# hooman007/ProtoASNet

Measured on AMD Instinct MI355X. Metric: clips/sec forward, higher is better.
Workload: dtype bf16; 1 GPU; Video ProtoASNet forward, x3d_s trunk + prototype layer (P=30, D=256, K=3), 32x16x224x224 echo clips per GPU; global_batch=32, parallelism=dp1 (independent clips, no collective), launch=hipGraph replay of the forward's launch list (one graph launch per step)

## Files before the change

### protoasnet_amd/csrc/stem_mfma.hip

```cpp
#include "common.h"
#include "igemm_epilogue.h"

namespace pasn {

constexpr int SM_ROWS = 4, SM_COLS = 56, SM_PC = 116, SM_PR = 2 * (SM_ROWS - 1) + 3, SM_RING = 6;
static_assert(SM_PC % 4 == 0 && SM_PC >= 2 * SM_COLS + 4, "whole 4-column staging units, every window inside the patch");
constexpr int SM_PF = 3;

template <typename TIN>
struct SmRaw;
template <>
struct SmRaw<float> {
    f32x4 v;
    __device__ void load(const float* p) { v = *reinterpret_cast<const f32x4*>(p); }
    __device__ float get(int e) const { return v[e]; }
};
template <>
struct SmRaw<__bf16> {
    bf16x4 v;
    __device__ void load(const __bf16* p) { v = *reinterpret_cast<const bf16x4*>(p); }
    __device__ float get(int e) const { return (float)v[e]; }
};
template <>
struct SmRaw<unsigned char> {
    unsigned v;
    __device__ void load(const unsigned char* p) { v = *reinterpret_cast<const unsigned*>(p); }
    __device__ float get(int e) const { return (float)((v >> (8 * e)) & 0xffu); }
};

template <typename TIN, int CIN>
__global__ __launch_bounds__(256, 2) void x3d_stem_mfma_kernel(const TIN* __restrict__ x, const __bf16* __restrict__ wq,
                                                               const float* __restrict__ scale, const float* __restrict__ bias,
                                                               __bf16* __restrict__ y, pasn_conv_desc d, float in_a, float in_b) {
    constexpr int NT = 1, MT = 2, BN = 32, OROW = BN + 8;
    constexpr int RPF = CIN * 3;
    constexpr int KROWS = 5 * RPF;
    constexpr int KS = (KROWS + 3) / 4;
    constexpr int SLOT = CIN * SM_PR * SM_PC;
    constexpr int UNITS = SLOT / 4;
    constexpr int UPT = (UNITS + 255) / 256;
    extern __shared__ __attribute__((aligned(16))) char smem[];
    __bf16* const ring = reinterpret_cast<__bf16*>(smem);
    __bf16* const imgs = reinterpret_cast<__bf16*>(smem + SM_RING * SLOT * 2);
    float* const scb = reinterpret_cast<float*>(smem + SM_RING * SLOT * 2 + 4 * 32 * OROW * 2);
    const int tid = threadIdx.x, lane = tid & 63, wave = __builtin_amdgcn_readfirstlane(tid >> 6);
    const int c = lane & 31, h = lane >> 5;
    const int T = d.Ti;

    const int ncol = (d.Wo + SM_COLS - 1) / SM_COLS, nrow = (d.Ho + SM_ROWS - 1) / SM_ROWS;
    int b = blockIdx.x;
    const int ct = b % ncol;
    b /= ncol;
    const int rt = b % nrow;
    const int n = b / nrow;
    const int oh0 = rt * SM_ROWS, ow0 = ct * SM_COLS;
    const int hi_base = oh0 * 2 - 1, wi_base = ow0 * 2 - 4;

    bf16x8 wa[KS];
#pragma unroll
    for (int s = 0; s < KS; ++s) wa[s] = *reinterpret_cast<const bf16x8*>(wq + ((size_t)(2 * s + h) * BN + c) * 8);
    igemm_stage_scale_bias<BN>(scb, scale, bias, 0, d.Cout_p, tid);

    const long plane = (long)d.Hi * d.Wi;
    int uoff[UPT];
    int uci[UPT];
#pragma unroll
    for (int k = 0; k < UPT; ++k) {
        const int u = tid + 256 * k;
        const int pc4 = u % (SM_PC / 4), r = (u / (SM_PC / 4)) % SM_PR, ci = u / ((SM_PC / 4) * SM_PR);
        const int hi = hi_base + r, wi = wi_base + pc4 * 4;
        const bool ok = u < UNITS && (unsigned)hi < (unsigned)d.Hi && (unsigned)wi < (unsigned)d.Wi;
        uoff[k] = ok ? hi * d.Wi + wi : -1;
        uci[k] = ci < CIN ? ci : CIN - 1;
    }
    SmRaw<TIN> raw[UPT];
    auto fetch = [&](int ti) {
#pragma unroll
        for (int k = 0; k < UPT; ++k)
            raw[k].load(x + (((long)n * CIN + uci[k]) * T + ti) * plane + (uoff[k] >= 0 ? uoff[k] : 0));
    };
    auto stage = [&](int slot, bool inside) {
        __bf16* dst = ring + slot * SLOT;
#pragma unroll
        for (int k = 0; k < UPT; ++k) {
            const int u = tid + 256 * k;
            float v[4];
#pragma unroll
            for (int e = 0; e < 4; ++e) v[e] = (inside && uoff[k] >= 0) ? fmaf(raw[k].get(e), in_a, in_b) : 0.0f;
            if (u < UNITS) store4(dst + u * 4, v);
        }
    };

    const int lane_off = (2 * wave) * SM_PC + 2 * c + 2;
    const int oh = oh0 + wave;
    const int cgs = d.Cout_p / 8;
    __bf16* const img = imgs + (size_t)wave * 32 * OROW;

    auto emit = [&](int to, const int (&sb)[5]) {
        f32x16 acc[NT][MT];
#pragma unroll
        for (int j = 0; j < MT; ++j)
#pragma unroll
            for (int r = 0; r < 16; ++r) acc[0][j][r] = 0.0f;
#pragma unroll
        for (int s = 0; s < KS; ++s) {
            auto rowoff = [&](int R) {
                const int Rc = R < KROWS ? R : KROWS - 1;
                return sb[Rc / RPF] + (((Rc % RPF) / 3) * SM_PR + (Rc % RPF) % 3) * SM_PC;
            };
            const int oa = h ? rowoff(4 * s + 2) : rowoff(4 * s + 0);
            const int ob = h ? rowoff(4 * s + 3) : rowoff(4 * s + 1);
            const __bf16* srca = ring + lane_off + oa;
            const __bf16* srcb = ring + lane_off + ob;
            bf16x8 bfr[MT];
#pragma unroll
            for (int j = 0; j < MT; ++j) {
                typedef unsigned u32x4 __attribute__((ext_vector_type(4)));
                const unsigned* pa = reinterpret_cast<const unsigned*>(srca + 64 * j);
                const unsigned* pb = reinterpret_cast<const unsigned*>(srcb + 64 * j);
                u32x4 v;
                v.x = pa[0];
                v.y = pa[1];
                v.z = pb[0];
                v.w = pb[1];
                bfr[j] = __builtin_bit_cast(bf16x8, v);
            }
#pragma unroll
            for (int j = 0; j < MT; ++j) mma32(acc[0][j], wa[s], bfr[j]);
        }
        __builtin_amdgcn_sched_group_barrier(0x100, 2 * MT * SM_PF, 0);
#pragma unroll
        for (int s = 0; s < KS; ++s) {
            __builtin_amdgcn_sched_group_barrier(0x008, MT, 0);
            if (s + SM_PF < KS) __builtin_amdgcn_sched_group_barrier(0x100, 2 * MT, 0);
        }
        igemm_epilogue<NT, MT>(acc, img, scb, nullptr, y, 0, cgs, d, lane, [&](int j, long& mbase, int& nvalid) {
            mbase = (((long)n * d.To + to) * d.Ho + oh) * d.Wo + ow0 + 32 * j;
            nvalid = oh < d.Ho ? min(min(32, SM_COLS - 32 * j), d.Wo - (ow0 + 32 * j)) : 0;
        });
    };

    const int nf = T + 4;
    int r = 0;
#pragma unroll 1
    for (int f = 0; f < nf; ++f) {
        const int ti = f - 2;
        stage(r, ti >= 0 && ti < T);
        if (ti + 1 >= 0 && ti + 1 < T) fetch(ti + 1);
        __syncthreads();
        const int to = f - 4;
        if (to >= 0) {
            int sb[5];
#pragma unroll
            for (int kt = 0; kt < 5; ++kt) {
                int q = r + 2 + kt;
                q = q >= SM_RING ? q - SM_RING : q;
                q = q >= SM_RING ? q - SM_RING : q;
                sb[kt] = q * SLOT;
            }
            emit(to, sb);
        }
        r = r + 1 == SM_RING ? 0 : r + 1;
    }
}

int x3d_stem_mfma_supported(const pasn_conv_desc& d, int out_dtype) {
    if (const char* e = tune("PASN_NO_STEM_MFMA"))
        if (e[0] == '1') return 0;
    if (out_dtype != PASN_BF16 || (d.Cin != 1 && d.Cin != 3) || d.Cout_p > 32) return 0;
    if (d.kt != 1 || d.kh != 3 || d.kw != 3 || d.st != 1 || d.sh != 2 || d.sw != 2 || d.pt != 0 || d.ph != 1 || d.pw != 1) return 0;
    if (d.Wi % 4 != 0 || d.To != d.Ti) return 0;
    if ((long)d.N * d.Cin * d.Ti * d.Hi * d.Wi >= (1L << 31)) return 0;
    return 1;
}

template <typename TIN>
static int launch_stem_mfma_t(const void* x, const void* wq, const float* scale, const float* bias, void* y, const pasn_conv_desc& d,
                              float in_a, float in_b, hipStream_t s) {
    const size_t slot = (size_t)d.Cin * SM_PR * SM_PC * 2;
    const size_t lds = SM_RING * slot + (size_t)4 * 32 * (32 + 8) * 2 + 32 * 8;
    const dim3 grid((unsigned)((long)d.N * ceil_div(d.Ho, SM_ROWS) * ceil_div(d.Wo, SM_COLS))), block(256);
    if (d.Cin == 3) {
        PASN_MAX_LDS(96 * 1024, x3d_stem_mfma_kernel<TIN, 3>);
        hipLaunchKernelGGL((x3d_stem_mfma_kernel<TIN, 3>), grid, block, lds, s, (const TIN*)x, (const __bf16*)wq, scale, bias, (__bf16*)y, d,
                           in_a, in_b);
    } else {
        hipLaunchKernelGGL((x3d_stem_mfma_kernel<TIN, 1>), grid, block, lds, s, (const TIN*)x, (const __bf16*)wq, scale, bias, (__bf16*)y, d,
                           in_a, in_b);
    }
    return check_launch("x3d_stem_mfma_kernel");
}

int launch_x3d_stem_mfma(const void* x, const void* wq, const float* scale, const float* bias, void* y, const pasn_conv_desc& d, int in_dtype,
                         float in_a, float in_b, hipStream_t s) {
    if (in_dtype == PASN_F32) return launch_stem_mfma_t<float>(x, wq, scale, bias, y, d, in_a, in_b, s);
    if (in_dtype == PASN_BF16) return launch_stem_mfma_t<__bf16>(x, wq, scale, bias, y, d, in_a, in_b, s);
    if (in_dtype == PASN_U8) return launch_stem_mfma_t<unsigned char>(x, wq, scale, bias, y, d, in_a, in_b, s);
    set_error("x3d_stem_mfma: unknown input dtype");
    return PASN_ERR_ARG;
}

}
```

### protoasnet_amd/csrc/x3d_edp.hip

```cpp
#include "common.h"
#include "xb_pointwise.h"

namespace pasn {

struct EdpArgs {
    const __bf16* x;
    const __bf16* w_a;
    const float *s_a, *b_a;
    const unsigned short* wq;
    const float *s_dw, *b_dw;
    const __bf16* w_c;
    const float *s_c, *b_c;
    __bf16* y;
    const __bf16* w_n;
    const float *s_n, *b_n;
    __bf16* e_next;
    int N, T, Cm, Cmp, Cxp, Cnp;
};

#ifdef PASN_TUNING
__device__ long long edp_stamps[8];
#define EDP_NOW() ((long long)__builtin_amdgcn_s_memrealtime())
#define EDP_ON (g.stamps && blockIdx.x == 0 && threadIdx.x == 0)
#endif

__device__ __forceinline__ void edp_barrier() { asm volatile("s_waitcnt lgkmcnt(0)\n\ts_barrier" ::: "memory"); }

constexpr int EDP_HW = 7, EDP_S = 49;
constexpr int EDP_RWI = 10, EDP_SLOTS = 10;
constexpr int EDP_ROWP = EDP_RWI * EDP_SLOTS + 2;
constexpr int EDP_FB = 9 * EDP_ROWP * 16;
constexpr int EDP_CPL = 9;

template <int KSA, int KSC, bool NEXT>
__global__ __launch_bounds__(512) void x3d_edp_kernel(EdpArgs a, EdpGeom g) {
    extern __shared__ __attribute__((aligned(1024))) char smem[];
    constexpr int XPL = 2 * KSA + 1;
    constexpr int TF = 2, NF = TF + 2, R = TF * EDP_S, RI = NF * EDP_S;
    const int lane = threadIdx.x & 63, wave = __builtin_amdgcn_readfirstlane(threadIdx.x >> 6);
    const int tid = threadIdx.x;
    const int c = lane & 31, h = lane >> 5;
    const int m = lane & 15, q4 = lane >> 4;
    char* const xin = smem;
    char* const fimg = smem + g.fimg_off;
    char* const dch = smem + g.dch_off;
    char* const xt = fimg;
    unsigned* const rowtab = reinterpret_cast<unsigned*>(smem + g.tab_off);
    float* const cst = reinterpret_cast<float*>(smem + g.cst_off);
    const int Cmp = a.Cmp, Cxp = a.Cxp, T = a.T;
    float* const sdw = cst, *const bdw = cst + Cmp, *const scp = cst + 2 * Cmp, *const bcp = scp + 32 * g.CTC, *const snp = bcp + 32 * g.CTC,
                *const bnp = snp + 32 * g.CTN;

#ifdef PASN_TUNING
    long long te = 0, td = 0, tp = 0, tq = 0;
    if (EDP_ON) edp_stamps[0] = EDP_NOW();
#endif
    for (int i = tid; i < (g.tab_off - g.fimg_off) / 16; i += 512) reinterpret_cast<uint4*>(fimg)[i] = uint4{0u, 0u, 0u, 0u};
    for (int i = tid; i < Cmp; i += 512) {
        sdw[i] = a.s_dw[i];
        bdw[i] = a.b_dw[i];
    }
    for (int i = tid; i < 32 * g.CTC; i += 512) {
        scp[i] = a.s_c[i];
        bcp[i] = a.b_c[i];
    }
    if (NEXT)
        for (int i = tid; i < 32 * g.CTN; i += 512) {
            snp[i] = a.s_n[i];
            bnp[i] = a.b_n[i];
        }
    const long M = (long)a.N * T * EDP_S;
    const __amdgpu_buffer_rsrc_t xrsrc = __builtin_amdgcn_make_buffer_rsrc(const_cast<__bf16*>(a.x), 0, (unsigned)(M * Cxp * 2), 0x00020000);
    const __amdgpu_buffer_rsrc_t yrsrc = __builtin_amdgcn_make_buffer_rsrc(a.y, 0, (unsigned)(M * Cxp * 2), 0x00020000);
    const __amdgpu_buffer_rsrc_t ersrc = __builtin_amdgcn_make_buffer_rsrc(NEXT ? a.e_next : a.y, 0, NEXT ? (unsigned)(M * a.Cnp * 2) : 0u, 0x00020000);
    const int PPR = Cxp >> 3;
    const int nTch = (T + TF - 1) / TF;
    const int lbl = xcd_remap(blockIdx.x, gridDim.x);
    const int tile_end = min(g.tiles, (lbl + 1) * g.tpb);
    const int ctw = wave & 3, tfo = wave >> 2;
    const int mrow = m / EDP_HW, mcol = m - mrow * EDP_HW;
    const int dwsel = (m & 7) >> 1, wsh = (m & 1) * 16;
    int tapoff[5];
#pragma unroll
    for (int j = 0; j < 5; ++j) {
        const int tap9 = min(2 * j + (q4 >> 1), 8);
        tapoff[j] = ((tap9 / 3) * EDP_ROWP + (tap9 % 3) * EDP_SLOTS) * 16;
    }
    const bool mpos = m < 2 * EDP_HW;
    const int lbase0 = ((mpos ? mrow : 1) * EDP_ROWP + (mpos ? mcol : EDP_HW - 1) * EDP_SLOTS + 2 * ctw + (q4 & 1)) * 16;
    constexpr int lstep = 2 * EDP_ROWP * 16;
    const int CT16 = (Cmp + 15) >> 4;
    const int prt = wave & 3, pcg = wave >> 2;
    const int ea = wave & 1, er = wave >> 1;
    __syncthreads();

#pragma unroll 1
    for (int tile = lbl * g.tpb; tile < tile_end; ++tile) {
        const int tch = tile % nTch, n = tile / nTch;
        const int t0 = tch * TF;
        const int nix = (RI * XPL + 63) >> 6;
        for (int j = wave; j < nix; j += 8) {
            const int s = j * 64 + lane;
            const int r = s / XPL, p = s - r * XPL;
            const int f = r / EDP_S, pos = r - f * EDP_S, ti = t0 - 1 + f;
            const unsigned off = (r < RI && p < PPR && ti >= 0 && ti < T) ? (unsigned)(((n * T + ti) * EDP_S + pos) * Cxp + p * 8) * 2u : XB_OOB;
            __builtin_amdgcn_raw_ptr_buffer_load_lds(xrsrc, (xb_lds_ptr_t)(xin + j * 1024), 16, (int)off, 0, 0, 0);
        }
        if (tid < 128) {
            const int f = tid / EDP_S, pos = tid - f * EDP_S;
            rowtab[tid] = (tid < R && t0 + f < T) ? (unsigned)((n * T + t0 + f) * EDP_S + pos) : 0xffffffffu;
        }
        f32x16 pacc[3];
#pragma unroll
        for (int i = 0; i < 3; ++i)
#pragma unroll
            for (int r = 0; r < 16; ++r) pacc[i][r] = 0.0f;
        asm volatile("s_waitcnt vmcnt(0)" ::: "memory");
        __syncthreads();
#ifdef PASN_TUNING
        if (EDP_ON) edp_stamps[1] = EDP_NOW();
#endif

#pragma unroll 1
        for (int qd = 0; qd < g.NQ; ++qd) {
#ifdef PASN_TUNING
            if (g.stamps) tq = EDP_NOW();
#endif
            {
                const int co = min(2 * qd + ea, g.CTA - 1);
                const bool colive = 2 * qd + ea < g.CTA;
                bf16x8 A[KSA];
                const __bf16* ab = a.w_a + ((long)co * KSA * 64 + lane) * 8;
#pragma unroll
                for (int ks = 0; ks < KSA; ++ks) A[ks] = load_frag<__bf16>(ab + ks * 512);
                float scv[2][8], bsv[2][8];
#pragma unroll
                for (int pr = 0; pr < 2; ++pr) {
                    load8(a.s_a + co * 32 + 16 * pr + 8 * h, scv[pr]);
                    load8(a.b_a + co * 32 + 16 * pr + 8 * h, bsv[pr]);
                }
                f32x16 acc[2];
#pragma unroll
                for (int i = 0; i < 2; ++i)
#pragma unroll
                    for (int r = 0; r < 16; ++r) acc[i][r] = 0.0f;
                const char* b0 = xin + ((er * 32 + c) * XPL + h) * 16;
#pragma unroll
                for (int ks = 0; ks < KSA; ++ks) {
                    const bf16x8 B0 = *reinterpret_cast<const bf16x8*>(b0 + ks * 32);
                    const bf16x8 B1 = *reinterpret_cast<const bf16x8*>(b0 + 4 * 32 * XPL * 16 + ks * 32);
                    acc[0] = __builtin_amdgcn_mfma_f32_32x32x16_bf16(A[ks], B0, acc[0], 0, 0, 0);
                    acc[1] = __builtin_amdgcn_mfma_f32_32x32x16_bf16(A[ks], B1, acc[1], 0, 0, 0);
                }
#pragma unroll
                for (int i = 0; i < 2; ++i) {
                    const int r = (er + 4 * i) * 32 + c;
                    const int f = r / EDP_S, pos = r - f * EDP_S;
                    const int ph = pos / EDP_HW, pw = pos - ph * EDP_HW;
                    const int ti = t0 - 1 + f;
                    const bool wr = colive && r < RI;
                    const bool inclip = ti >= 0 && ti < T;
                    char* const cell = wr ? fimg + f * EDP_FB + ((ph + 1) * EDP_ROWP + (pw + 1) * EDP_SLOTS + 4 * ea + h) * 16 : dch + R * EDP_CPL * 16;
#pragma unroll
                    for (int pr = 0; pr < 2; ++pr) {
                        float v[8];
#pragma unroll
                        for (int qq = 0; qq < 4; ++qq) {
                            const auto sw = __builtin_amdgcn_permlane32_swap(__float_as_uint(acc[i][8 * pr + qq]), __float_as_uint(acc[i][8 * pr + 4 + qq]), false, false);
                            v[qq] = __uint_as_float(sw[0]);
                            v[4 + qq] = __uint_as_float(sw[1]);
                        }
#pragma unroll
                        for (int e = 0; e < 8; ++e) v[e] = v[e] * scv[pr][e] + bsv[pr][e];
                        bf16x8 o;
#pragma unroll
                        for (int e = 0; e < 8; ++e) o[e] = (__bf16)relu_f32(v[e]);
                        xb_u32x4 ou = __builtin_bit_cast(xb_u32x4, o);
                        if (!inclip) ou = xb_u32x4{0u, 0u, 0u, 0u};
                        *reinterpret_cast<xb_u32x4*>(cell + (wr ? pr * 32 : 0)) = ou;
                    }
                }
            }
            const int c0 = (qd * 4 + ctw) * 16;
            const bool dlive = c0 < Cmp;
            const int ct = min(qd * 4 + ctw, CT16 - 1);
            const uint4* wp = reinterpret_cast<const uint4*>(a.wq + ((size_t)(ct * 2) * 64 + lane) * 8);
            const uint4 w0v = wp[0], w1v = wp[64];
            bf16x8 PA[3][4];
#pragma unroll
            for (int i = 0; i < 3; ++i)
#pragma unroll
                for (int kk = 0; kk < 4; ++kk)
                    PA[i][kk] = load_frag<__bf16>(a.w_c + ((long)((pcg + 2 * i) * KSC + min(4 * qd + kk, KSC - 1)) * 64 + lane) * 8);
            edp_barrier();
#ifdef PASN_TUNING
            if (g.stamps) {
                const long long now = EDP_NOW();
                te += now - tq;
                tq = now;
            }
#endif
            if (dlive && t0 + tfo < T) {
                xb_u32x4 A[3][5];
                const unsigned wd[8] = {w0v.x, w0v.y, w0v.z, w0v.w, w1v.x, w1v.y, w1v.z, w1v.w};
#pragma unroll
                for (int kt = 0; kt < 3; ++kt)
#pragma unroll
                    for (int j = 0; j < 5; ++j) {
                        const int e = kt * 5 + j;
                        const unsigned bits = ((e & 1) ? (wd[e >> 1] >> 16) : (wd[e >> 1] & 0xffffu)) << wsh;
                        A[kt][j] = xb_u32x4{dwsel == 0 ? bits : 0u, dwsel == 1 ? bits : 0u, dwsel == 2 ? bits : 0u, dwsel == 3 ? bits : 0u};
                    }
                f32x4 S[4];
#pragma unroll
                for (int l = 0; l < 4; ++l) S[l] = f32x4{0.0f, 0.0f, 0.0f, 0.0f};
#pragma unroll
                for (int kt = 0; kt < 3; ++kt) {
                    const char* fb = fimg + (tfo + kt) * EDP_FB + lbase0;
#pragma unroll
                    for (int l = 0; l < 4; ++l) {
                        bf16x8 B[5];
#pragma unroll
                        for (int j = 0; j < 5; ++j) B[j] = *reinterpret_cast<const bf16x8*>(fb + tapoff[j] + l * lstep);
#pragma unroll
                        for (int j = 0; j < 5; ++j) S[l] = __builtin_amdgcn_mfma_f32_16x16x32_bf16(__builtin_bit_cast(bf16x8, A[kt][j]), B[j], S[l], 0, 0, 0);
                    }
                }
                const int ce = c0 + 4 * q4, cel = ctw * 16 + 4 * q4;
                const bool cev = ce < Cmp;
                const f32x4 s4 = *reinterpret_cast<const f32x4*>(sdw + min(ce, Cmp - 4)), b4 = *reinterpret_cast<const f32x4*>(bdw + min(ce, Cmp - 4));
#pragma unroll
                for (int l = 0; l < 4; ++l) {
                    const int lr = 2 * l + mrow;
                    const bool ok = m < 2 * EDP_HW && lr < EDP_HW && cev;
                    float v[4];
#pragma unroll
                    for (int i = 0; i < 4; ++i) {
                        v[i] = S[l][i] * (cev ? s4[i] : 0.0f) + (cev ? b4[i] : 0.0f);
                        v[i] = v[i] * sigmoidf_(v[i]);
                    }
                    bf16x4 o;
#pragma unroll
                    for (int i = 0; i < 4; ++i) o[i] = (__bf16)v[i];
                    const int r = ok ? tfo * EDP_S + lr * EDP_HW + mcol : R;
                    *reinterpret_cast<bf16x4*>(dch + (r * EDP_CPL) * 16 + (ok ? cel : 0) * 2) = o;
                }
            }
            edp_barrier();
#ifdef PASN_TUNING
            if (g.stamps) {
                const long long now = EDP_NOW();
                td += now - tq;
                tq = now;
            }
#endif
            {
                const char* b0 = dch + ((prt * 32 + c) * EDP_CPL + h) * 16;
#pragma unroll
                for (int kk = 0; kk < 4; ++kk) {
                    if (4 * qd + kk < KSC) {
                        const bf16x8 B = *reinterpret_cast<const bf16x8*>(b0 + kk * 32);
#pragma unroll
                        for (int i = 0; i < 3; ++i) pacc[i] = __builtin_amdgcn_mfma_f32_32x32x16_bf16(PA[i][kk], B, pacc[i], 0, 0, 0);
                    }
                }
            }
#ifdef PASN_TUNING
            if (g.stamps) tp += EDP_NOW() - tq;
#endif
        }
#ifdef PASN_TUNING
        if (EDP_ON) {
            edp_stamps[2] = EDP_NOW();
            edp_stamps[5] = te;
            edp_stamps[6] = td;
            edp_stamps[7] = tp;
        }
#endif
        if (NEXT) __syncthreads();
        {
            const int r = prt * 32 + c;
            const unsigned gp = rowtab[r];
#pragma unroll
            for (int i = 0; i < 3; ++i) {
                const int co = pcg + 2 * i;
                unsigned off[2];
                uint4 rraw[2];
#pragma unroll
                for (int pr = 0; pr < 2; ++pr) {
                    const int ch = co * 32 + 16 * pr + 8 * h;
                    off[pr] = (gp != 0xffffffffu && ch < Cxp) ? (gp * (unsigned)Cxp + (unsigned)ch) * 2u : XB_OOB;
                    rraw[pr] = __builtin_bit_cast(uint4, __builtin_amdgcn_raw_buffer_load_b128(xrsrc, (int)off[pr], 0, 0));
                }
#pragma unroll
                for (int pr = 0; pr < 2; ++pr) {
                    float v[8], r8[8], scv[8], bsv[8];
#pragma unroll
                    for (int qq = 0; qq < 4; ++qq) {
                        const auto sw = __builtin_amdgcn_permlane32_swap(__float_as_uint(pacc[i][8 * pr + qq]), __float_as_uint(pacc[i][8 * pr + 4 + qq]), false, false);
                        v[qq] = __uint_as_float(sw[0]);
                        v[4 + qq] = __uint_as_float(sw[1]);
                    }
                    const int ch = co * 32 + 16 * pr + 8 * h;
                    load8(scp + ch, scv);
                    load8(bcp + ch, bsv);
                    const uint4 rr1[1] = {rraw[pr]};
                    raw_to_f8<__bf16>(rr1, r8);
#pragma unroll
                    for (int e = 0; e < 8; ++e) v[e] = v[e] * scv[e] + bsv[e];
#pragma unroll
                    for (int e = 0; e < 8; ++e) v[e] += r8[e];
                    bf16x8 o;
#pragma unroll
                    for (int e = 0; e < 8; ++e) o[e] = (__bf16)relu_f32(v[e]);
                    __builtin_amdgcn_raw_buffer_store_b128(__builtin_bit_cast(xb_u32x4, o), yrsrc, (int)off[pr], 0, 0);
                    if (NEXT && ch < Cxp) *reinterpret_cast<bf16x8*>(xt + (r * XPL + (ch >> 3)) * 16) = o;
                }
            }
        }
#ifdef PASN_TUNING
        if (EDP_ON) edp_stamps[3] = EDP_NOW();
#endif
        if (NEXT) {
            __syncthreads();
            xb_pointwise<KSA, 4, false, false>(a.w_n, snp, bnp, xt, XPL, g.CTN, 4, rowtab, ersrc, ersrc, a.Cnp, nullptr, 0, wave, lane);
            __syncthreads();
#ifdef PASN_TUNING
            if (EDP_ON) edp_stamps[4] = EDP_NOW();
#endif
            for (int i = tid; i < (NF * EDP_FB) / 16; i += 512) reinterpret_cast<uint4*>(fimg)[i] = uint4{0u, 0u, 0u, 0u};
        }
        __syncthreads();
    }
}

static bool edp_pointwise(const pasn_conv_desc& d) {
    return d.kt == 1 && d.kh == 1 && d.kw == 1 && d.st == 1 && d.sh == 1 && d.sw == 1 && !d.pt && !d.ph && !d.pw;
}

EdpGeom edp_geom(const pasn_conv_desc& da, const pasn_conv_desc& dd, const pasn_conv_desc& dc, const pasn_conv_desc* dn, int dtype) {
    EdpGeom g{};
    if (dtype != PASN_BF16) return g;
    if (const char* e = tune("PASN_NO_EDP"))
        if (e[0] == '1') return g;
    const bool stencil = dd.kt == 3 && dd.kh == 3 && dd.kw == 3 && dd.st == 1 && dd.sh == 1 && dd.sw == 1 && dd.pt == 1 && dd.ph == 1 && dd.pw == 1 &&
                         dd.To == dd.Ti && dd.Ho == dd.Hi && dd.Wo == dd.Wi && dd.Cin_p == dd.Cout_p && dd.act == PASN_ACT_SWISH;
    if (!stencil || !edp_pointwise(da) || !edp_pointwise(dc) || da.act != PASN_ACT_RELU || dc.act != PASN_ACT_RELU || da.in_swish || dc.in_swish) return g;
    if (dd.Hi != EDP_HW || dd.Wi != EDP_HW) return g;
    if (da.N != dd.N || da.To != dd.Ti || da.Ho != dd.Hi || da.Wo != dd.Wi || da.Cout != dd.Cin || da.Cout_p != dd.Cin_p) return g;
    if (dc.N != dd.N || dc.To != dd.To || dc.Ho != dd.Ho || dc.Wo != dd.Wo || dc.Cin != dd.Cout || dc.Cin_p != dd.Cout_p) return g;
    if (dc.Cout != da.Cin || dc.Cout_p != da.Cin_p) return g;
    if (da.w_frag != 1 || dc.w_frag != 1 || da.Cin_p != 192 || dd.Cout_p != 432) return g;
    g.KSA = da.Cin_p / 16;
    g.KSC = (dd.Cout_p + 31) / 32 * 2;
    if (da.w_kc != g.KSA * 16 || dc.w_kc != g.KSC * 16) return EdpGeom{};
    g.CTA = (da.Cout_p + 31) / 32;
    g.CTC = (dc.Cout_p + 31) / 32;
    if (g.CTC != 6 || da.w_rows < g.CTA * 32 || dc.w_rows < g.CTC * 32) return EdpGeom{};
    if (dn) {
        if (!edp_pointwise(*dn) || dn->act != PASN_ACT_RELU || dn->in_swish || dn->w_frag != 1) return EdpGeom{};
        if (dn->N != dc.N || dn->To != dc.To || dn->Ho != dc.Ho || dn->Wo != dc.Wo || dn->Cin != dc.Cout || dn->Cin_p != dc.Cout_p) return EdpGeom{};
        g.CTN = (dn->Cout_p + 31) / 32;
        if (dn->w_kc != g.KSA * 16 || dn->w_rows < g.CTN * 32 || dn->Cout_p % 8) return EdpGeom{};
    }
    const long M = (long)dd.N * dd.To * EDP_S;
    if (M * dd.Cout_p * 2 >= (1L << 30) || (dn && M * dn->Cout_p * 2 >= (1L << 30))) return EdpGeom{};
    g.NQ = ceil_div(dd.Cout_p, 64);
    auto kib = [](int b) { return (b + 1023) / 1024 * 1024; };
    const int xpl = 2 * g.KSA + 1;
    g.fimg_off = kib(4 * EDP_S * xpl * 16);
    const int fimg_bytes = kib(std::max(4 * EDP_FB, dn ? 128 * xpl * 16 + 64 : 0));
    g.dch_off = g.fimg_off + fimg_bytes;
    g.tab_off = g.dch_off + kib((2 * EDP_S + 1) * EDP_CPL * 16 + 64);
    g.cst_off = g.tab_off + 1024;
    g.lds_bytes = g.cst_off + kib((2 * dd.Cout_p + 64 * g.CTC + 64 * g.CTN) * 4);
    if (g.lds_bytes > 160 * 1024) return EdpGeom{};
    g.tiles = dd.N * ceil_div(dd.To, 2);
    const int grid = std::min(g.tiles, 256);
    g.tpb = ceil_div(g.tiles, grid);
    g.grid = ceil_div(g.tiles, g.tpb);
    g.stamps = tune_dev("PASN_EDP_STAMPS") ? 1 : 0;
    g.ok = 1;
    return g;
}

}

using namespace pasn;

#ifdef PASN_TUNING
extern "C" int pasn_debug_edp_stamps(long long* host_out) { return (int)hipMemcpyFromSymbol(host_out, HIP_SYMBOL(pasn::edp_stamps), sizeof(long long) * 8); }
#endif

static bool edp_desc_ok(const pasn_conv_desc* d) { return d && d->N > 0 && d->To > 0 && d->Ho > 0 && d->Wo > 0 && d->Cin > 0 && d->Cout > 0; }

extern "C" int pasn_x3d_edp_supported(const pasn_conv_desc* d_a, const pasn_conv_desc* d_dw, const pasn_conv_desc* d_c, const pasn_conv_desc* d_n, int dtype) {
    if (!edp_desc_ok(d_a) || !edp_desc_ok(d_dw) || !edp_desc_ok(d_c) || (d_n && !edp_desc_ok(d_n))) return 0;
    return edp_geom(*d_a, *d_dw, *d_c, d_n, dtype).ok;
}

extern "C" int pasn_x3d_edp_fwd(const void* x, const void* w_a, const float* scale_a, const float* bias_a, const void* w_dw, const float* scale_dw,
                                const float* bias_dw, const void* w_c, const float* scale_c, const float* bias_c, void* y, const void* w_n,
                                const float* scale_n, const float* bias_n, void* e_next, const pasn_conv_desc* d_a, const pasn_conv_desc* d_dw,
                                const pasn_conv_desc* d_c, const pasn_conv_desc* d_n, int dtype, void* stream) {
    PASN_REQUIRE(x && w_a && scale_a && bias_a && w_dw && scale_dw && bias_dw && w_c && scale_c && bias_c && y, "null pointer");
    PASN_REQUIRE((d_n != nullptr) == (w_n != nullptr) && (d_n == nullptr || (scale_n && bias_n && e_next)), "the next expand conv comes with all of its operands, or not at all");
    PASN_REQUIRE(edp_desc_ok(d_a) && edp_desc_ok(d_dw) && edp_desc_ok(d_c) && (!d_n || edp_desc_ok(d_n)), "bad geometry");
    const EdpGeom g = edp_geom(*d_a, *d_dw, *d_c, d_n, dtype);
    PASN_REQUIRE(g.ok, "block not covered (pasn_x3d_edp_supported returns 0)");
    EdpArgs a{(const __bf16*)x, (const __bf16*)w_a, scale_a, bias_a, (const unsigned short*)w_dw, scale_dw, bias_dw, (const __bf16*)w_c, scale_c, bias_c,
              (__bf16*)y, (const __bf16*)w_n, scale_n, bias_n, (__bf16*)e_next, d_dw->N, d_dw->To, d_dw->Cout, d_dw->Cout_p, d_a->Cin_p,
              d_n ? d_n->Cout_p : 0};
    const dim3 grid(g.grid), block(512);
    if (d_n) {
        PASN_MAX_LDS(160 * 1024, x3d_edp_kernel<12, 28, true>);
        hipLaunchKernelGGL((x3d_edp_kernel<12, 28, true>), grid, block, (size_t)g.lds_bytes, (hipStream_t)stream, a, g);
    } else {
        PASN_MAX_LDS(160 * 1024, x3d_edp_kernel<12, 28, false>);
        hipLaunchKernelGGL((x3d_edp_kernel<12, 28, false>), grid, block, (size_t)g.lds_bytes, (hipStream_t)stream, a, g);
    }
    return check_launch("x3d_edp_kernel");
}
```

Before: 12020 clips/s.

## Prime stem ring early, overlap EDP input fetch with setup, reuse staged residual

```diff
diff --git a/protoasnet_amd/csrc/stem_mfma.hip b/protoasnet_amd/csrc/stem_mfma.hip
--- a/protoasnet_amd/csrc/stem_mfma.hip
+++ b/protoasnet_amd/csrc/stem_mfma.hip
@@ -48,7 +48,7 @@
     const int T = d.Ti;
 
     const int ncol = (d.Wo + SM_COLS - 1) / SM_COLS, nrow = (d.Ho + SM_ROWS - 1) / SM_ROWS;
-    int b = blockIdx.x;
+    int b = xcd_remap(blockIdx.x, gridDim.x);
     const int ct = b % ncol;
     b /= ncol;
     const int rt = b % nrow;
@@ -74,12 +74,12 @@
         uci[k] = ci < CIN ? ci : CIN - 1;
     }
     SmRaw<TIN> raw[UPT];
-    auto fetch = [&](int ti) {
+    auto fetch = [&](SmRaw<TIN>(&raw)[UPT], int ti) {
 #pragma unroll
         for (int k = 0; k < UPT; ++k)
             raw[k].load(x + (((long)n * CIN + uci[k]) * T + ti) * plane + (uoff[k] >= 0 ? uoff[k] : 0));
     };
-    auto stage = [&](int slot, bool inside) {
+    auto stage = [&](const SmRaw<TIN>(&raw)[UPT], int slot, bool inside) {
         __bf16* dst = ring + slot * SLOT;
 #pragma unroll
         for (int k = 0; k < UPT; ++k) {
@@ -140,16 +140,25 @@
         });
     };
 
+    static_assert((4 * SLOT) % 16 == 0, "slots 0 and 1 cleared in 16-byte units");
+    for (int i = tid; i < (4 * SLOT) / 16; i += 256) reinterpret_cast<uint4*>(ring)[i] = uint4{0u, 0u, 0u, 0u};
+    {
+        SmRaw<TIN> raw0[UPT], raw1[UPT];
+        fetch(raw0, 0);
+        if (1 < T) fetch(raw1, 1);
+        if (2 < T) fetch(raw, 2);
+        stage(raw0, 2, true);
+        stage(raw1, 3, 1 < T);
+        stage(raw, 4, 2 < T);
+    }
+    if (3 < T) fetch(raw, 3);
+    __syncthreads();
     const int nf = T + 4;
-    int r = 0;
+    int r = 4;
 #pragma unroll 1
-    for (int f = 0; f < nf; ++f) {
-        const int ti = f - 2;
-        stage(r, ti >= 0 && ti < T);
-        if (ti + 1 >= 0 && ti + 1 < T) fetch(ti + 1);
-        __syncthreads();
-        const int to = f - 4;
-        if (to >= 0) {
+    for (int f = 4;;) {
+        {
+            const int to = f - 4;
             int sb[5];
 #pragma unroll
             for (int kt = 0; kt < 5; ++kt) {
@@ -161,6 +170,11 @@
             emit(to, sb);
         }
         r = r + 1 == SM_RING ? 0 : r + 1;
+        if (++f == nf) break;
+        const int ti = f - 2;
+        stage(raw, r, ti < T);
+        if (ti + 1 < T) fetch(raw, ti + 1);
+        __syncthreads();
     }
 }
 
diff --git a/protoasnet_amd/csrc/x3d_edp.hip b/protoasnet_amd/csrc/x3d_edp.hip
--- a/protoasnet_amd/csrc/x3d_edp.hip
+++ b/protoasnet_amd/csrc/x3d_edp.hip
@@ -55,20 +55,6 @@
     long long te = 0, td = 0, tp = 0, tq = 0;
     if (EDP_ON) edp_stamps[0] = EDP_NOW();
 #endif
-    for (int i = tid; i < (g.tab_off - g.fimg_off) / 16; i += 512) reinterpret_cast<uint4*>(fimg)[i] = uint4{0u, 0u, 0u, 0u};
-    for (int i = tid; i < Cmp; i += 512) {
-        sdw[i] = a.s_dw[i];
-        bdw[i] = a.b_dw[i];
-    }
-    for (int i = tid; i < 32 * g.CTC; i += 512) {
-        scp[i] = a.s_c[i];
-        bcp[i] = a.b_c[i];
-    }
-    if (NEXT)
-        for (int i = tid; i < 32 * g.CTN; i += 512) {
-            snp[i] = a.s_n[i];
-            bnp[i] = a.b_n[i];
-        }
     const long M = (long)a.N * T * EDP_S;
     const __amdgpu_buffer_rsrc_t xrsrc = __builtin_amdgcn_make_buffer_rsrc(const_cast<__bf16*>(a.x), 0, (unsigned)(M * Cxp * 2), 0x00020000);
     const __amdgpu_buffer_rsrc_t yrsrc = __builtin_amdgcn_make_buffer_rsrc(a.y, 0, (unsigned)(M * Cxp * 2), 0x00020000);
@@ -76,26 +62,8 @@
     const int PPR = Cxp >> 3;
     const int nTch = (T + TF - 1) / TF;
     const int lbl = xcd_remap(blockIdx.x, gridDim.x);
-    const int tile_end = min(g.tiles, (lbl + 1) * g.tpb);
-    const int ctw = wave & 3, tfo = wave >> 2;
-    const int mrow = m / EDP_HW, mcol = m - mrow * EDP_HW;
-    const int dwsel = (m & 7) >> 1, wsh = (m & 1) * 16;
-    int tapoff[5];
-#pragma unroll
-    for (int j = 0; j < 5; ++j) {
-        const int tap9 = min(2 * j + (q4 >> 1), 8);
-        tapoff[j] = ((tap9 / 3) * EDP_ROWP + (tap9 % 3) * EDP_SLOTS) * 16;
-    }
-    const bool mpos = m < 2 * EDP_HW;
-    const int lbase0 = ((mpos ? mrow : 1) * EDP_ROWP + (mpos ? mcol : EDP_HW - 1) * EDP_SLOTS + 2 * ctw + (q4 & 1)) * 16;
-    constexpr int lstep = 2 * EDP_ROWP * 16;
-    const int CT16 = (Cmp + 15) >> 4;
-    const int prt = wave & 3, pcg = wave >> 2;
-    const int ea = wave & 1, er = wave >> 1;
-    __syncthreads();
-
-#pragma unroll 1
-    for (int tile = lbl * g.tpb; tile < tile_end; ++tile) {
+    const int tile0 = lbl * g.tpb, tile_end = min(g.tiles, (lbl + 1) * g.tpb);
+    auto request_x = [&](int tile) {
         const int tch = tile % nTch, n = tile / nTch;
         const int t0 = tch * TF;
         const int nix = (RI * XPL + 63) >> 6;
@@ -110,6 +78,43 @@
             const int f = tid / EDP_S, pos = tid - f * EDP_S;
             rowtab[tid] = (tid < R && t0 + f < T) ? (unsigned)((n * T + t0 + f) * EDP_S + pos) : 0xffffffffu;
         }
+    };
+    if (tile0 < tile_end) request_x(tile0);
+    for (int i = tid; i < (g.tab_off - g.fimg_off) / 16; i += 512) reinterpret_cast<uint4*>(fimg)[i] = uint4{0u, 0u, 0u, 0u};
+    for (int i = tid; i < Cmp; i += 512) {
+        sdw[i] = a.s_dw[i];
+        bdw[i] = a.b_dw[i];
+    }
+    for (int i = tid; i < 32 * g.CTC; i += 512) {
+        scp[i] = a.s_c[i];
+        bcp[i] = a.b_c[i];
+    }
+    if (NEXT)
+        for (int i = tid; i < 32 * g.CTN; i += 512) {
+            snp[i] = a.s_n[i];
+            bnp[i] = a.b_n[i];
+        }
+    const int ctw = wave & 3, tfo = wave >> 2;
+    const int mrow = m / EDP_HW, mcol = m - mrow * EDP_HW;
+    const int dwsel = (m & 7) >> 1, wsh = (m & 1) * 16;
+    int tapoff[5];
+#pragma unroll
+    for (int j = 0; j < 5; ++j) {
+        const int tap9 = min(2 * j + (q4 >> 1), 8);
+        tapoff[j] = ((tap9 / 3) * EDP_ROWP + (tap9 % 3) * EDP_SLOTS) * 16;
+    }
+    const bool mpos = m < 2 * EDP_HW;
+    const int lbase0 = ((mpos ? mrow : 1) * EDP_ROWP + (mpos ? mcol : EDP_HW - 1) * EDP_SLOTS + 2 * ctw + (q4 & 1)) * 16;
+    constexpr int lstep = 2 * EDP_ROWP * 16;
+    const int CT16 = (Cmp + 15) >> 4;
+    const int prt = wave & 3, pcg = wave >> 2;
+    const int ea = wave & 1, er = wave >> 1;
+
+#pragma unroll 1
+    for (int tile = tile0; tile < tile_end; ++tile) {
+        const int tch = tile % nTch;
+        const int t0 = tch * TF;
+        if (tile != tile0) request_x(tile);
         f32x16 pacc[3];
 #pragma unroll
         for (int i = 0; i < 3; ++i)
@@ -290,7 +295,7 @@
                 for (int pr = 0; pr < 2; ++pr) {
                     const int ch = co * 32 + 16 * pr + 8 * h;
                     off[pr] = (gp != 0xffffffffu && ch < Cxp) ? (gp * (unsigned)Cxp + (unsigned)ch) * 2u : XB_OOB;
-                    rraw[pr] = __builtin_bit_cast(uint4, __builtin_amdgcn_raw_buffer_load_b128(xrsrc, (int)off[pr], 0, 0));
+                    rraw[pr] = *reinterpret_cast<const uint4*>(xin + ((EDP_S + r) * XPL + min(ch >> 3, XPL - 1)) * 16);
                 }
 #pragma unroll
                 for (int pr = 0; pr < 2; ++pr) {
@@ -324,13 +329,17 @@
         if (NEXT) {
             __syncthreads();
             xb_pointwise<KSA, 4, false, false>(a.w_n, snp, bnp, xt, XPL, g.CTN, 4, rowtab, ersrc, ersrc, a.Cnp, nullptr, 0, wave, lane);
+#ifdef PASN_TUNING
+            if (EDP_ON) edp_stamps[4] = EDP_NOW();
+#endif
+        }
+        if (tile + 1 < tile_end) {
+            if (NEXT) {
+                __syncthreads();
+                for (int i = tid; i < (NF * EDP_FB) / 16; i += 512) reinterpret_cast<uint4*>(fimg)[i] = uint4{0u, 0u, 0u, 0u};
+            }
             __syncthreads();
-#ifdef PASN_TUNING
-            if (EDP_ON) edp_stamps[4] = EDP_NOW();
-#endif
-            for (int i = tid; i < (NF * EDP_FB) / 16; i += 512) reinterpret_cast<uint4*>(fimg)[i] = uint4{0u, 0u, 0u, 0u};
-        }
-        __syncthreads();
+        }
     }
 }
 
```

New measurement: 12100 clips/s, median of 6. No clear change (+0.7%).
